# jonaselgammal/GPry

Measured on AMD Instinct MI355X. Metric: gp_refit_plus_nora_acq_cycle_throughput, higher is better.
Workload: dtype f64

## Files before the change

gpry_amd/_lib.py:

```python
import ctypes as C
import ctypes as _ct
import os

import numpy as np

_HERE = os.path.dirname(os.path.abspath(__file__))
LIB_PATH = os.path.join(_HERE, "libgpry_hip.so")

GPRY_MAX_DIM = 32
MASK_CLASSIFIED_INF = 1
MASK_OUTSIDE_TRUST = 2

KERNEL_IDS = {"rbf": 0, "matern12": 1, "matern32": 2, "matern52": 3}
KERNEL_WHITE = 0x10


class GpryAffine(C.Structure):
    _fields_ = [("has_x_affine", C.c_int),
                ("x_lo", C.c_double * GPRY_MAX_DIM),
                ("x_span", C.c_double * GPRY_MAX_DIM),
                ("y_mean", C.c_double), ("y_std", C.c_double),
                ("clip_hi", C.c_double)]


# ... 56 lines not shown
                                + [C.c_int, C.c_int, _vp, _vp]),
    "gpry_maximize_mean": (C.c_int, [_vp, _vp, _vp, _vp, _vp, C.c_int64, _vp, _vp, C.c_int, C.c_int, C.c_double,
                                     C.c_double, C.c_double] + [_vp] * 12 + [_P(C.c_double)]),
    "gpry_maximize_acq": (C.c_int, [_vp, _vp, _vp, _vp, C.c_int64, _vp, _vp, C.c_double, C.c_double, C.c_double, C.c_int,
                                    C.c_int, C.c_double, C.c_double, C.c_double] + [_vp] * 14 + [_P(C.c_double)]),
    "gpry_hessian_mean": (C.c_int, [_vp, _vp, C.c_int64, _vp, _vp, _vp, _P(C.c_double)]),
    "gpry_predict_cov": (C.c_int, [_vp, _vp, C.c_int64, _vp, _vp, _vp, _P(C.c_double)]),
    "gpry_sample_joint": (C.c_int, [_vp, _vp, C.c_int64, _vp, C.c_int64, C.c_uint64, C.c_double, _vp, _vp, _vp, _vp,
                                    _P(C.c_int), _P(C.c_double), _P(C.c_double)]),
    "gpry_loo": (C.c_int, [_vp, _vp, _vp, _vp, _vp, _vp, _P(C.c_double)]),
    "gpry_svm_fit": (C.c_int, [_vp, _vp, _vp, C.c_int64, C.c_int64, C.c_double, C.c_double, C.c_double, C.c_int64, _vp,
                               _P(C.c_double), _P(C.c_double), _P(C.c_double), _P(C.c_int64), _P(C.c_int), _P(C.c_double)]),
    "gpry_leave_out": (C.c_int, [_vp, _vp, _vp, C.c_int64, _vp, _vp, _vp, _vp, _vp, _P(C.c_double)]),
    "gpry_predict_grad": (C.c_int, [_vp, _vp, C.c_int, _vp, _vp, _vp]),
    "gpry_predict_grad_batch": (C.c_int, [_vp, _vp, C.c_int64, C.c_int, _vp, _vp, _vp, _vp]),
    "gpry_predict_point": (C.c_int, [_vp, _vp, C.c_int, C.c_int, _vp, _vp, _vp, _vp, _vp]),
    "gpry_set_gates": (C.c_int, [_vp, _vp, _vp, C.c_int64, C.c_double, C.c_double, C.c_int, _vp]),
    "gpry_sweep_logexp": (C.c_int, [_vp, _vp, C.c_int64, _vp, C.c_double, C.c_double,
                                    C.c_double, _vp, _vp, _vp, _P(C.c_int64)]),
    "gpry_sweep_logexp_given": (C.c_int, [_vp, _vp, C.c_int64, _vp, _vp, _vp, C.c_double, C.c_double,
                                          C.c_double, _vp, _vp, _vp, _P(C.c_int64)]),
    "gpry_sweep_fetch": (C.c_int, [_vp, C.c_int64, _vp, _vp, _vp]),
    "gpry_sweep_prune_info": (C.c_int, [_vp, _vp, _vp]),
    "gpry_sweep_topk": (C.c_int, [_vp, C.c_int64, _vp, C.c_int64, _vp, _P(C.c_int64),
                                  _P(C.c_double)]),
    "gpry_kb_reset": (C.c_int, [_vp]),
    "gpry_kb_register": (C.c_int, [_vp, _vp, C.c_int64, _P(C.c_int64), _vp]),
    "gpry_kb_gram": (C.c_int, [_vp, C.c_int64, _vp, _vp, _P(C.c_int64)]),
    "gpry_kb_gram_rows": (C.c_int, [_vp, _vp, C.c_int64, _vp, _vp, _P(C.c_int64)]),
    "gpry_kb_rank": (C.c_int, [_vp, _vp, C.c_int64, _vp, C.c_int64, _vp, _vp, _vp, _vp, C.c_int64, _vp, C.c_int64, _vp,
                               C.c_int64, _vp, _vp, _vp, _vp, _vp, _P(C.c_int64), _P(C.c_int64), _vp]),
    "gpry_comm_unique_id": (C.c_int, [_vp]),
    "gpry_comm_init": (C.c_int, [_vp, C.c_int, C.c_int, _vp, _P(_vp)]),
    "gpry_comm_destroy": (C.c_int, [_vp]),
    "gpry_comm_info": (C.c_int, [_vp, _P(C.c_int), _P(C.c_int), _P(C.c_int)]),
    "gpry_comm_allgather": (C.c_int, [_vp, _vp, C.c_int64, _vp]),
    "gpry_comm_allreduce_max": (C.c_int, [_vp, _vp, C.c_int64]),
    "gpry_comm_barrier": (C.c_int, [_vp]),
    "gpry_group_create": (C.c_int, [C.c_int, _P(C.c_int), _vp, _P(_vp)]),
    "gpry_group_destroy": (C.c_int, [_vp]),
    "gpry_group_size": (C.c_int, [_vp, _P(C.c_int), _P(C.c_int)]),
    "gpry_group_member": (_vp, [_vp, C.c_int]),
    "gpry_group_last_error": (C.c_char_p, [_vp]),
    "gpry_group_set_model": (C.c_int, [_vp, _vp, _vp, _vp, C.c_int64, C.c_int, C.c_int, _vp,
                                       _P(GpryAffine), _P(C.c_int)]),
    "gpry_group_set_gates": (C.c_int, [_vp, _vp, _vp, C.c_int64, C.c_double, C.c_double, C.c_int, _vp]),
# ... 686 lines not shown
        self._check(self._lib.gpry_sweep_info(self._h, C.byref(form), _ptr(est)), "gpry_sweep_info")
        return {"panel_form": self.PANEL_FORMS.get(form.value, str(form.value)), "panel_error_estimate": float(est[0]),
                "panel_error_mean_worst_case": float(est[1]), "panel_error_variance": float(est[2]), "panel_gate": float(est[3])}

    def sweep_fetch(self, want=("y", "sigma")):
        M = self._sweep_M
        out = {k: (np.empty(M) if k in want else None) for k in ("y", "sigma", "acq")}
        self._check(self._lib.gpry_sweep_fetch(self._h, M, _ptr(out["y"]), _ptr(out["sigma"]),
                                               _ptr(out["acq"])), "gpry_sweep_fetch")
        return out

    PRUNE_INFO = ("pruned", "M", "K_prime", "rounds", "contracted", "completed", "K", "survivors", "y_bound", "live_blocks",
                  "blocks")

    def sweep_prune_info(self):
        info = np.zeros(len(self.PRUNE_INFO), dtype=np.int64)
        dinfo = np.zeros(5)
        self._check(self._lib.gpry_sweep_prune_info(self._h, _ptr(info), _ptr(dinfo)), "gpry_sweep_prune_info")
        out = {k: int(v) for k, v in zip(self.PRUNE_INFO, info)}
        out["tau"] = float(dinfo[0])
        out["stage_ms"] = dict(zip(("sweep_mean", "sweep_prune_select", "sweep_compact", "sweep_prune_gemm"), dinfo[1:].tolist()))
        return out

    def sweep_topk(self, Kp, exclude=None):
        Kp = int(Kp)
        top = np.zeros(max(Kp, 1), dtype=CAND_DTYPE)
        n_out, bound = C.c_int64(0), C.c_double(0.0)
        if exclude is not None and len(exclude):
            exclude = np.ascontiguousarray(np.sort(np.asarray(exclude, dtype=np.int64)))
            nex = len(exclude)
        else:
            exclude, nex = None, 0
        self._check(self._lib.gpry_sweep_topk(self._h, Kp, _ptr(exclude), nex, _ptr(top),
                                              C.byref(n_out), C.byref(bound)), "gpry_sweep_topk")
        return top[:n_out.value], bound.value

    def kb_reset(self):
        self._check(self._lib.gpry_kb_reset(self._h), "gpry_kb_reset")

    def kb_register(self, X, want_var0=True):
        X = _f64(X)
        m = X.shape[0]
        first = C.c_int64(0)
        var0 = np.empty(m) if want_var0 else None
        self._check(self._lib.gpry_kb_register(self._h, _ptr(X), m, C.byref(first), _ptr(var0)),
                    "gpry_kb_register")
# ... 256 lines not shown
```

gpry_amd/csrc/common.h:

```cpp
#pragma once
#include <hip/hip_runtime.h>
#include <stdint.h>
#include <stdio.h>
#include <string.h>
#include <math.h>
#include <string>
#include <vector>
#include <map>

#include "../../include/gpry_hip.h"

#define GPRY_THETA_MAX (2 + GPRY_MAX_DIM)
#define GPRY_BPAR_ROW (2 + GPRY_MAX_DIM)
#define GPRY_BPAR_WHITE (1 + GPRY_MAX_DIM)
#define GPRY_TILE 128
#define GPRY_NB 64

typedef double v4d __attribute__((ext_vector_type(4)));

struct StageTimer {
    double total_ms = 0.0;
    int64_t count = 0;
    std::vector<std::pair<hipEvent_t, hipEvent_t>> pending;
};
// ... 99 lines not shown
    double* dG = nullptr;
    int64_t g_cap = 0;
    double* dsplit = nullptr;
    int64_t split_cap = 0;
    int opt_predict_split = 1;
    int opt_gemm_dma = 1;
    double* dpart = nullptr;
    int64_t part_cap = 0;
    unsigned long long* dkeys = nullptr; int64_t keys_cap = 0;
    unsigned int* dhist = nullptr;
    unsigned int* dselp = nullptr;
    enum { SELP_HIST_WORDS = 12 * 256, SELP_WORDS = 12 * 256 + 12 * 8 };
    int opt_select_fused = 1;
    int opt_prune_one_select = 1;
    int opt_sweep_small_map = 1;
    gpry_cand* dcand = nullptr; int64_t cand_cap = 0;
    unsigned long long* dsel = nullptr;
    enum { DSEL_NAN = 0,
           DSEL_STATE = 0,
           DSEL_EMIT = 4,
           DSEL_SURV = 6,
           DSEL_GIDX = 7,
           DSEL_LIVE = 8,
           DSEL_WORDS = 64 };

    int64_t kb_n = 0, kb_cap = 0;
    int64_t kb_ld = 0;
    double* dU = nullptr;
    double* dXkb = nullptr;
    double* dkbout = nullptr;

    double* dbord = nullptr;
    int64_t bord_cap = 0;
    int64_t n_border = 0;

    void* trtri_plan = nullptr;
    void* trtri_pipe = nullptr;
    int64_t opt_gemm_streamk = 5632;
    int64_t opt_topk_host = 16384;
    int opt_factor_pipeline = 1;
    int opt_factor_pipeline_min = 1280;
    void* chol_plan = nullptr;

    void* srv = nullptr;
    int opt_predict_serve = 1;
    int64_t opt_serve_idle_us = 2000;
    int opt_mcmc_mapped = 0;
    int64_t opt_chol_stacked = 2048;
    int opt_chol_stacked_dense = 0;
    int opt_sweep_overlap = 0;
    int opt_sweep_upload = 1;
    const double* up_X = nullptr;
    const double* up_y = nullptr;
    int up_gates = 0;
    int opt_kb_rank = 1;
    int opt_predict_gates = 0;
    int opt_sweep_prune = 0;
    int opt_sweep_mean_bound = 1;
    int sw_pruned = 0;
    struct PruneState {
        int have_mask = 0;
        int form = 0;
        FinishParams fp = {};
        int64_t n_eval = 0;
        int64_t rounds = 0, evaluated_total = 0, completed = 0, last_K = 0;
        int64_t n_gidx = 0;
        int tau_done = 0;
        double tau = 0.0;
        int64_t survivors = -1;
        int ybound = 0;
        int64_t live_blocks = 0, blocks = 0;
    } prune;
    struct ModelSnap {
        double *dV = nullptr, *dalpha_ = nullptr, *dXs = nullptr, *dX = nullptr;
        int64_t v_cap = 0, a_cap = 0, xs_cap = 0, x_cap = 0;
        int64_t N = 0, Np = 0;
        int d = 0, dpad = 0, kernel_id = 0;
        bool white = false;
        double theta[GPRY_THETA_MAX] = {0};
        gpry_affine tf;
        double xcenter[GPRY_MAX_DIM] = {0};
        bool xs_foreign = false;
    } snap;
    double* dub = nullptr;
    int64_t ub_cap = 0;
    double* dXg = nullptr;
    int64_t xg_cap = 0;
    int64_t* dgidx = nullptr;
    int64_t gidx_cap = 0;
    uint8_t* dmc = nullptr;
    int64_t mc_cap = 0;
    uint8_t* dknn = nullptr;
    int64_t knn_cap = 0;
    uint8_t* dph = nullptr;
// ... 214 lines not shown
```

gpry_amd/csrc/ctx.hip:

```cpp
#include "common.h"
#include <string>
#include <stdarg.h>
#include <dlfcn.h>

thread_local char g_last_error[1024] = {0};
void trtri_plan_free(gpry_ctx* ctx);
void overlap_plan_free(gpry_ctx* ctx);

int gpry_fail(gpry_ctx* ctx, int code, const char* fmt, ...) {
    va_list ap;
    va_start(ap, fmt);
    vsnprintf(g_last_error, sizeof(g_last_error), fmt, ap);
    va_end(ap);
    if (ctx) { strncpy(ctx->err, g_last_error, sizeof(ctx->err) - 1); }
    return code;
}

template <typename T>
int dev_alloc(gpry_ctx* ctx, T** p, int64_t count) {
    *p = nullptr;
    if (count <= 0) count = 1;
    HIP_TRY(ctx, hipMalloc((void**)p, sizeof(T) * (size_t)count));
    return 0;
}
// ... 246 lines not shown
    OPT_INT("gemm_streamk", opt_gemm_streamk, 0, BIG, trtri_plan_free(c)),
    OPT_INT("gemm_small", opt_gemm_small, 0, BIG, c->lml_cache = false),
    OPT_INT("cross_mfma", opt_cross_mfma, 0, 1, (void)0),
    OPT_INT("cross_hybrid", opt_cross_hybrid, 0, 1, (void)0),
    OPT_INT("sweep_chunk", opt_sweep_chunk, 0, BIG, c->opt_sweep_chunk = round_up(c->opt_sweep_chunk, 1024)),
    OPT_INT("topk_host", opt_topk_host, 0, BIG, (void)0),
    OPT_INT("lml_small", opt_lml_small, 0, 1, c->lml_cache = false),
    OPT_INT("lml_cache", opt_lml_cache, 0, 1, c->lml_cache = false),
    OPT_INT("lml_batch", opt_lml_batch, 0, BIG, (void)0),
    OPT_INT("lml_batch_mb", opt_lml_batch_mb, 1, BIG, (void)0),
    OPT_INT("lml_schedule", opt_lml_schedule, 0, 1, (void)0),
    OPT_INT("lml_streams", opt_lml_streams, 1, 8, (void)0),
    OPT_INT("chol_tp_segments", opt_chol_tp_segments, 0, 1, c->lml_cache = false),
    OPT_INT("panel_debug", opt_panel_debug, 0, 511, c->lml_cache = false),
    OPT_INT("tp_left", opt_tp_left, 0, 1, (void)0),
    OPT_INT("tp_block", opt_tp_block, 128, BIG, c->opt_tp_block = round_up(c->opt_tp_block, 128); overlap_plan_free(c)),
    OPT_INT("tp_tail", opt_tp_tail, 128, BIG, c->opt_tp_tail = round_up(c->opt_tp_tail, 128); overlap_plan_free(c)),
    OPT_INT("predict_small", opt_predict_small, 0, BIG, (void)0),
    OPT_INT("predict_split", opt_predict_split, 0, 1, (void)0),
    OPT_INT("sweep_upload", opt_sweep_upload, 0, 1, (void)0),
    OPT_INT("sweep_overlap", opt_sweep_overlap, 0, 1, (void)0),
    OPT_INT("sweep_prune", opt_sweep_prune, 0, 1, (void)0),
    OPT_INT("sweep_mean_bound", opt_sweep_mean_bound, 0, 1, (void)0),
    OPT_INT("sweep_small_map", opt_sweep_small_map, 0, 1, (void)0),
    OPT_INT("select_fused", opt_select_fused, 0, 1, (void)0),
    OPT_INT("prune_one_select", opt_prune_one_select, 0, 1, (void)0),
    OPT_INT("chol_stacked", opt_chol_stacked, 0, BIG, c->lml_cache = false),
    OPT_INT("chol_stacked_dense", opt_chol_stacked_dense, 0, 1, c->lml_cache = false),
    OPT_INT("predict_gates", opt_predict_gates, 0, 1, (void)0),
    OPT_INT("predict_serve", opt_predict_serve, 0, 1, (void)0),
    OPT_INT("serve_idle_us", opt_serve_idle_us, 10, 1000000, (void)0),
    OPT_INT("mcmc_mapped", opt_mcmc_mapped, 0, 1, (void)0),
    OPT_INT("kb_rank", opt_kb_rank, 0, 1, (void)0),
    OPT_INT("svm_iters_per_launch", opt_svm_iters, 1, BIG, (void)0),
};
#undef OPT_INT
const OptionSpec* find_option(const char* key) {
    for (const OptionSpec& o : OPTIONS) if (!strcmp(o.key, key)) return &o;
    return nullptr;
}
}

int gpry_ctx_set_option(gpry_ctx* ctx, const char* key, int64_t value) {
    if (!ctx || !key) return gpry_fail(ctx, -1, "gpry_ctx_set_option: NULL argument");
    GPRY_TRY(serve_stop(ctx));
    const OptionSpec* o = find_option(key);
// ... 374 lines not shown
```

gpry_amd/csrc/kernel_build.hip:

```cpp
#include "common.h"

#include "kern_math.h"

__global__ void scale_train_kernel(const double* __restrict__ X, double* __restrict__ Xs_,
                                   int64_t N, int64_t Np, int d, int dpad, AffParams ap, int* info_,
                                   const double* __restrict__ bpar, int64_t bstride) {
    const int tb = (int)blockIdx.z;
    double* __restrict__ Xs = bset(Xs_, tb, bstride);
    int* info = bset(info_, tb, bstride);
    int64_t idx = (int64_t)blockIdx.x * blockDim.x + threadIdx.x;
    if (idx < 4) info[idx] = 0;
    if (idx >= Np * dpad) return;
    int64_t i = idx / dpad; int k = (int)(idx - i * dpad);
    double v = 0.0;
    if (i < N && k < d) v = X[i * d + k] / (bpar ? bset(bpar, tb, bstride)[1 + k] : ap.ls[k]);
    Xs[idx] = v;
}

int launch_scale_train(gpry_ctx* ctx) {
    AffParams ap = make_ap(ctx, false);
    int64_t n = ctx->Np * ctx->dpad;
    hipLaunchKernelGGL(scale_train_kernel, dim3((unsigned)((n + 255) / 256), 1, (unsigned)ctx->bn), dim3(256), 0,
                       ctx->stream, ctx->dX, ctx->dXs, ctx->N, ctx->Np, ctx->d, ctx->dpad, ap, ctx->dinfo, ctx->bpar, ctx->bstride);
    HIP_TRY(ctx, hipGetLastError());
// ... 223 lines not shown
    for (int jj = nfull; jj < 128; jj++) {
        double v = 0.0;
        if (jj < nvalid) {
            double r2 = 0.0;
#pragma unroll
            for (int k = 0; k < DP; k++) {
                double df = xs[k] - Xl[jj * DP + k];
                r2 = fma(df, df, r2);
            }
            v = kp.C * corr_r2_fast<KID>(r2);
            macc = fma(al[jj], v, macc);
        }
        if (in_chunk && Kst) Kst[((int64_t)jc * 128 + jj) * ldk + ml] = v;
    }
    if (in_chunk && mean_part) mean_part[(int64_t)jc * mc + ml] = macc;
}

template <int DP, int KID, bool HYB, bool BND = false>
__global__ __launch_bounds__(256) void cross_build_mfma_kernel(
    const double* __restrict__ Xcs, int64_t ldm, int64_t mc,
    const double* __restrict__ Ycs, const double* __restrict__ alpha_,
    double* __restrict__ Kst, int64_t ldk, double* __restrict__ mean_part, KernParams kp, double ucut,
    double ubnd = 0.0, double uhi = 0.0, double* __restrict__ sabs_part = nullptr,
    unsigned long long* __restrict__ live_cnt = nullptr) {
    constexpr int S = DP + 2, KS = DP / 4;
    constexpr double SC = corr_scale<KID>();
    __shared__ __attribute__((aligned(16))) double Yl[128 * S];
    __shared__ double yn[128], al[128];
    const int t = threadIdx.x, lane = t & 63, w = t >> 6, r = lane & 15, g = lane >> 4;
    const int jc = blockIdx.y;
    const int64_t mb = (int64_t)blockIdx.x * 256 + 64 * w;
    for (int e = t; e < 128 * (DP / 2); e += 256) {
        const int row = e / (DP / 2), k2 = (e - row * (DP / 2)) * 2;
        *reinterpret_cast<double2*>(Yl + row * S + k2) = *reinterpret_cast<const double2*>(Ycs + ((int64_t)jc * 128 + row) * DP + k2);
    }
    if (t < 128) al[t] = alpha_ ? alpha_[jc * 128 + t] : 0.0;
    double xb[4][KS], xn[4];
#pragma unroll
    for (int tp = 0; tp < 2; tp++) {
        double s0 = 0.0, s1 = 0.0;
#pragma unroll
        for (int kk = 0; kk < KS; kk++) {
            const double2 v = *reinterpret_cast<const double2*>(Xcs + (int64_t)(4 * kk + g) * ldm + mb + 32 * tp + 2 * r);
            xb[2 * tp][kk] = v.x; xb[2 * tp + 1][kk] = v.y;
            s0 = fma(v.x, v.x, s0); s1 = fma(v.y, v.y, s1);
        }
        s0 += __shfl_xor(s0, 16); s0 += __shfl_xor(s0, 32);
        s1 += __shfl_xor(s1, 16); s1 += __shfl_xor(s1, 32);
        xn[2 * tp] = s0 * SC; xn[2 * tp + 1] = s1 * SC;
    }
    __syncthreads();
    if (t < 128) {
        double s = 0.0;
#pragma unroll
        for (int k = 0; k < DP; k++) s = fma(Yl[t * S + k], Yl[t * S + k], s);
        yn[t] = s * SC;
    }
    __syncthreads();
    const int64_t left = kp.N - (int64_t)jc * 128;
    const int nvalid = left >= 128 ? 128 : (left > 0 ? (int)left : 0);
    double macc[4] = {0.0, 0.0, 0.0, 0.0};
    double sacc[4] = {0.0, 0.0, 0.0, 0.0};
    unsigned nlive = 0;
#pragma unroll 1
    for (int j0 = 0; j0 < 128; j0 += 16) {
        double a[KS], ynq[4], alq[4];
#pragma unroll
        for (int kk = 0; kk < KS; kk++) a[kk] = Yl[(j0 + r) * S + 4 * kk + g];
#pragma unroll
        for (int q = 0; q < 4; q++) { ynq[q] = yn[j0 + g + 4 * q]; alq[q] = al[j0 + g + 4 * q]; }
#pragma unroll
        for (int tp = 0; tp < 2; tp++) {
            v4d acc0 = {0.0, 0.0, 0.0, 0.0}, acc1 = {0.0, 0.0, 0.0, 0.0};
#pragma unroll
            for (int kk = 0; kk < KS; kk++) acc0 = __builtin_amdgcn_mfma_f64_16x16x4f64(a[kk], xb[2 * tp][kk], acc0, 0, 0, 0);
#pragma unroll
            for (int kk = 0; kk < KS; kk++) acc1 = __builtin_amdgcn_mfma_f64_16x16x4f64(a[kk], xb[2 * tp + 1][kk], acc1, 0, 0, 0);
            const int64_t mloc = mb + 32 * tp + 2 * r;
            const bool in_chunk = mloc < mc;
            double ue0[4], ue1[4];
            bool live = false;
#pragma unroll
            for (int q = 0; q < 4; q++) {
                ue0[q] = fma(-2.0 * SC, acc0[q], xn[2 * tp] + ynq[q]);
                ue1[q] = fma(-2.0 * SC, acc1[q], xn[2 * tp + 1] + ynq[q]);
                if (BND) live = live || !(ue0[q] >= ubnd && ue0[q] <= uhi) || !(ue1[q] >= ubnd && ue1[q] <= uhi);
            }
            if (BND) {
                if (!__any(live)) continue;
                nlive++;
            }
#pragma unroll
            for (int q = 0; q < 4; q++) {
                const int jj = j0 + g + 4 * q;
                double u0 = ue0[q];
                double u1 = ue1[q];
                if (HYB && (u0 < ucut || u1 < ucut)) {
                    double r0 = 0.0, r1 = 0.0;
#pragma unroll 2
                    for (int k = 0; k < DP; k++) {
                        const double yk = Yl[jj * S + k];
                        const double2 xk = *reinterpret_cast<const double2*>(Xcs + (int64_t)k * ldm + mloc);
                        const double d0 = xk.x - yk, d1 = xk.y - yk;
                        r0 = fma(d0, d0, r0); r1 = fma(d1, d1, r1);
                    }
                    u0 = r0 * SC; u1 = r1 * SC;
                }
                u0 = fmax(u0, 1e-290);
                u1 = fmax(u1, 1e-290);
                double v0 = kp.C * corr_scaled_fast<KID>(u0);
                double v1 = kp.C * corr_scaled_fast<KID>(u1);
                if (jj >= nvalid) { v0 = 0.0; v1 = 0.0; }
// ... 4 lines not shown
                    sacc[2 * tp + 1] = fma(fabs(alq[q]), fabs(v1), sacc[2 * tp + 1]);
                }
                if (in_chunk && Kst) *reinterpret_cast<double2*>(Kst + ((int64_t)jc * 128 + jj) * ldk + mloc) = make_double2(v0, v1);
            }
        }
    }
    if (mean_part) {
#pragma unroll
        for (int tl = 0; tl < 4; tl++) {
            double s = macc[tl];
            s += __shfl_xor(s, 16);
            s += __shfl_xor(s, 32);
            const int64_t ml = mb + 32 * (tl >> 1) + 2 * r + (tl & 1);
            if (g == 0 && ml < mc) mean_part[(int64_t)jc * mc + ml] = s;
            if (BND) {
                double sa = sacc[tl];
                sa += __shfl_xor(sa, 16);
                sa += __shfl_xor(sa, 32);
                if (g == 0 && ml < mc) sabs_part[(int64_t)jc * mc + ml] = sa;
            }
        }
    }
    if (BND && lane == 0 && nlive) atomicAdd(live_cnt, (unsigned long long)nlive);
}
__global__ __launch_bounds__(256) void center_train_kernel(const double* __restrict__ X, double* __restrict__ Ycs, int64_t N, int64_t Np, int d,
                                                           int dsel, AffParams ap, AffParams cen) {
    const int64_t idx = (int64_t)blockIdx.x * blockDim.x + threadIdx.x;
    if (idx >= Np * dsel) return;
    const int64_t i = idx / dsel;
    const int k = (int)(idx - i * dsel);
    Ycs[idx] = (i < N && k < d) ? (X[i * d + k] - cen.lo[k]) / ap.ls[k] : 0.0;
}
__global__ __launch_bounds__(256) void center_cand_kernel(const double* __restrict__ Xc, int64_t M, int64_t m0, int64_t mc, int d, int dsel,
                                                          int has_aff, AffParams ap, AffParams cen, double* __restrict__ Xcs, int64_t ldm) {
    const int64_t idx = (int64_t)blockIdx.x * blockDim.x + threadIdx.x;
    if (idx >= mc * dsel) return;
    const int64_t ml = idx / dsel;
    const int k = (int)(idx - ml * dsel);
    const int64_t m = m0 + ml;
    double v = 0.0;
    if (k < d && m < M) {
        v = Xc[m * d + k];
        if (has_aff) v = (v - ap.lo[k]) / ap.span[k];
        v = (v - cen.lo[k]) / ap.ls[k];
    }
    Xcs[(int64_t)k * ldm + ml] = v;
// ... 40 lines not shown
                            int raw_affine, int hybrid) {
    hipStream_t st = ctx->stream;
    KernParams kp;
    int dsel = 0;
    int64_t ldm = 0;
    GPRY_TRY(center_cands(ctx, Xc, m0, mc, raw_affine, &kp, &dsel, &ldm));
    dim3 grid((unsigned)((mc + 255) / 256), (unsigned)(ctx->Np / 128));
#define CM2(DP, KID) do { const double ucut = 100.0 * corr_scale<KID>();                                                                  \
                       if (hybrid) { hipLaunchKernelGGL((cross_build_mfma_kernel<DP, KID, true>), grid, dim3(256), 0, st, ctx->dXcs, ldm, mc, ctx->dYcs, \
                                                        ctx->dalpha_, Kst, ldk, mean_part, kp, ucut); }                                  \
                       else { hipLaunchKernelGGL((cross_build_mfma_kernel<DP, KID, false>), grid, dim3(256), 0, st, ctx->dXcs, ldm, mc, ctx->dYcs, \
                                                 ctx->dalpha_, Kst, ldk, mean_part, kp, ucut); } } while (0)
#define CM4(KID) { if (dsel == 4) CM2(4, KID); else if (dsel == 8) CM2(8, KID); else if (dsel == 16) CM2(16, KID); \
                   else if (dsel == 24) CM2(24, KID); else CM2(32, KID); }
    DISPATCH_KID(ctx->kernel_id, CM4)
#undef CM4
#undef CM2
    HIP_TRY(ctx, hipGetLastError());
    return 0;
}

int launch_cross_mean_bound(gpry_ctx* ctx, const double* Xc, int64_t m0, int64_t mc, double* mean_part, double* sabs_part,
                            double ubnd, double uhi, unsigned long long* live_cnt) {
    hipStream_t st = ctx->stream;
    KernParams kp;
    int dsel = 0;
    int64_t ldm = 0;
    GPRY_TRY(center_cands(ctx, Xc, m0, mc, 1, &kp, &dsel, &ldm));
    dim3 grid((unsigned)((mc + 255) / 256), (unsigned)(ctx->Np / 128));
#define CB2(DP, KID) hipLaunchKernelGGL((cross_build_mfma_kernel<DP, KID, true, true>), grid, dim3(256), 0, st, ctx->dXcs, ldm, mc, ctx->dYcs, \
                                        ctx->dalpha_, nullptr, mc, mean_part, kp, 100.0 * corr_scale<KID>(), ubnd, uhi, sabs_part, live_cnt)
#define CB4(KID) { if (dsel == 4) CB2(4, KID); else if (dsel == 8) CB2(8, KID); else if (dsel == 16) CB2(16, KID); \
                   else if (dsel == 24) CB2(24, KID); else CB2(32, KID); }
    DISPATCH_KID(ctx->kernel_id, CB4)
#undef CB4
#undef CB2
    HIP_TRY(ctx, hipGetLastError());
    return 0;
}

template <int DP, int KID>
__global__ __launch_bounds__(256) void cross_build_small_kernel(
    const double* __restrict__ Xc, int64_t M, int64_t m0, int64_t mc,
    const double* __restrict__ Xs, const double* __restrict__ alpha_,
    double* __restrict__ Kst, int64_t ldk, double* __restrict__ mean_part,
    KernParams kp, AffParams ap) {
    __shared__ double Xl[128 * DP];
    __shared__ double al[128];
    const int t = threadIdx.x, rg = t >> 6;
    const int64_t ml = (int64_t)blockIdx.x * 64 + (t & 63);
    const int64_t m = m0 + ml;
    const int jc = blockIdx.y;
    for (int e = t; e < 128 * DP; e += 256) {
        int row = e / DP, k = e - row * DP;
// ... 786 lines not shown
```

gpry_amd/csrc/sweep.hip:

```cpp
#include "sweep.h"
#include "acq_math.h"
#include <algorithm>

__global__ void logexp_kernel(const double* __restrict__ mu, const double* __restrict__ sd, int64_t n, double zeta,
                              double baseline, double sigma_n, double* __restrict__ acq) {
    int64_t i = (int64_t)blockIdx.x * blockDim.x + threadIdx.x;
    if (i < n) acq[i] = logexp_value(mu[i], sd[i], zeta, baseline, sigma_n);
}
int launch_logexp(gpry_ctx* ctx, const double* mu, const double* sd, int64_t n, double zeta, double baseline, double sigma_n, double* acq) {
    hipLaunchKernelGGL(logexp_kernel, dim3((unsigned)((n + 255) / 256)), dim3(256), 0, ctx->stream, mu, sd, n, zeta, baseline, sigma_n, acq);
    HIP_TRY(ctx, hipGetLastError());
    return 0;
}

__device__ __forceinline__ double sum_partials(const double* __restrict__ part, int nt, int64_t ldp, int64_t col) {
    double s = 0.0;
#pragma unroll 8
    for (int t = 0; t < nt; t++) s += part[(int64_t)t * ldp + col];
    return s;
}
__device__ __forceinline__ double finish_y(double mu_, unsigned mk, const FinishParams& fp) {
    double y = mu_ * fp.y_std + fp.y_mean;
    y = fmin(y, fp.clip_hi);
    if (mk) y = -INFINITY;
// ... 285 lines not shown

int run_sweep(gpry_ctx* ctx, int64_t M, const SweepRequest& rq) {
    const bool predict = rq.kind == SWEEP_PREDICT, stage_a = rq.kind == SWEEP_STAGE_A, y_given = rq.y_given;
    const int64_t Np = ctx->Np;
    const int nt = (int)(Np / 128);
    const int64_t chunk = sweep_chunk(ctx, M);
    const bool overlap = ctx->opt_sweep_overlap && ctx->stream2 != nullptr && rq.kind == SWEEP_FULL && M > chunk;
    const int nbuf = overlap ? 2 : 1;
    if (stage_a) GPRY_TRY(dev_grow(ctx, &ctx->dub, &ctx->ub_cap, round_up(M, 1024)));
    else GPRY_TRY(dev_grow(ctx, &ctx->dKst, &ctx->kst_cap, nbuf * Np * chunk));
    const bool small_build = predict && M <= 512;
    const int nt_mean = small_build ? 4 * nt : nt;
    const int64_t part_stride = (int64_t)(nt_mean + nt) * chunk;
    GPRY_TRY(ensure_part(ctx, nbuf * part_stride));
    const FinishParams fp = finish_params(ctx, rq);
    ctx->sw_M = M;
    GPRY_TRY(choose_panel_form(ctx, small_build));
    const int form = ctx->panel_form;
    const bool no_panel = stage_a && y_given;
    if (panel_from_matrix_pipe(form) && !no_panel) GPRY_TRY(launch_cross_prepare(ctx));
    if (stage_a) ctx->prune.form = form;
    const MeanBound mb = mean_bound_setup(ctx, rq, fp, nt);
    unsigned long long* live_cnt = nullptr;
    if (stage_a) { ctx->prune.ybound = mb.on ? 1 : 0; ctx->prune.live_blocks = 0; ctx->prune.blocks = 0; }
    if (mb.on) {
        if (!ctx->dsel) GPRY_TRY(dev_alloc(ctx, &ctx->dsel, gpry_ctx::DSEL_WORDS));
        live_cnt = ctx->dsel + gpry_ctx::DSEL_LIVE;
        HIP_TRY(ctx, hipMemsetAsync(live_cnt, 0, 8, ctx->stream));
        if (getenv("GPRY_HIP_DEBUG_PANEL"))
            fprintf(stderr, "gpry: bound pass: u in [%.6g, %.3g] skipped, D %.3g, gamma %.3g\n", mb.ubnd, mb.uhi, mb.D1, mb.g3 / 3.0);
    }
    const double* up_X = ctx->up_X;
    const double* up_y = ctx->up_y;
    const size_t nchunk = (size_t)((M + chunk - 1) / chunk);
    if (up_X || overlap) {
        while (ctx->ev_pool.size() < 3 * nchunk + 1) {
            hipEvent_t ev;
            HIP_TRY(ctx, hipEventCreateWithFlags(&ev, hipEventDisableTiming));
            ctx->ev_pool.push_back(ev);
        }
    }
    const hipStream_t main_stream = ctx->stream, side = ctx->stream2;
    struct StreamSwap {
        gpry_ctx* c; hipStream_t keep;
        StreamSwap(gpry_ctx* ctx, hipStream_t st) : c(ctx), keep(ctx->stream) { c->stream = st; }
        ~StreamSwap() { c->stream = keep; }
    };
    auto upload_chunk = [&](size_t ci, bool gates_on_side) -> int {
        const int64_t m0 = (int64_t)ci * chunk, mc = (M - m0 < chunk) ? M - m0 : chunk;
        HIP_TRY(ctx, hipMemcpyAsync(ctx->dXc + m0 * ctx->d, up_X + m0 * ctx->d, sizeof(double) * mc * ctx->d,
                                    hipMemcpyHostToDevice, side));
// ... 189 lines not shown
    HIP_TRY(ctx, hipMemsetAsync(ctx->dsel + gpry_ctx::DSEL_GIDX, 0, 8, ctx->stream));
    hipLaunchKernelGGL(pruned_idx_kernel, dim3((unsigned)((M + 255) / 256)), dim3(256), 0, ctx->stream, ctx->dsig_all, M, ctx->dgidx, ctx->dsel + gpry_ctx::DSEL_GIDX);
    HIP_TRY(ctx, hipGetLastError());
    unsigned long long n = 0;
    HIP_TRY(ctx, hipMemcpyAsync(&n, ctx->dsel + gpry_ctx::DSEL_GIDX, 8, hipMemcpyDeviceToHost, ctx->stream));
    HIP_TRY(ctx, hipStreamSynchronize(ctx->stream));
    if (n > 0) GPRY_TRY(prune_eval(ctx, (int64_t)n));
    HIP_TRY(ctx, hipStreamSynchronize(ctx->stream));
    ctx->prune.evaluated_total += (int64_t)n;
    ctx->sw_pruned = 0;
    ctx->prune.completed = 1;
    return 0;
}

static int sweep_copy_out(gpry_ctx* ctx, int64_t M, const double* nan_src, unsigned long long* nn, unsigned long long* live,
                          double* y_all, double* sigma_all, double* acq_all) {
    if (nan_src) {
        if (!ctx->dsel) GPRY_TRY(dev_alloc(ctx, &ctx->dsel, gpry_ctx::DSEL_WORDS));
        unsigned long long* dnan = ctx->dsel + gpry_ctx::DSEL_NAN;
        HIP_TRY(ctx, hipMemsetAsync(dnan, 0, 8, ctx->stream));
        hipLaunchKernelGGL(count_nan_kernel, dim3(1024), dim3(256), 0, ctx->stream, nan_src, M, dnan);
        HIP_TRY(ctx, hipMemcpyAsync(nn, dnan, 8, hipMemcpyDeviceToHost, ctx->stream));
    }
    if (live) HIP_TRY(ctx, hipMemcpyAsync(live, ctx->dsel + gpry_ctx::DSEL_LIVE, 8, hipMemcpyDeviceToHost, ctx->stream));
    if (y_all) HIP_TRY(ctx, hipMemcpyAsync(y_all, ctx->dy_all, sizeof(double) * M, hipMemcpyDeviceToHost, ctx->stream));
    if (sigma_all) HIP_TRY(ctx, hipMemcpyAsync(sigma_all, ctx->dsig_all, sizeof(double) * M, hipMemcpyDeviceToHost, ctx->stream));
    if (acq_all) HIP_TRY(ctx, hipMemcpyAsync(acq_all, ctx->dacq_all, sizeof(double) * M, hipMemcpyDeviceToHost, ctx->stream));
    HIP_TRY(ctx, hipStreamSynchronize(ctx->stream));
    return 0;
}

static int sweep_impl(gpry_ctx* ctx, const double* X, int64_t M, const uint8_t* mask, const double* y_given, double zeta,
                      double baseline, double sigma_n, double* y_all, double* sigma_all, double* acq_all, int64_t* n_nan) {
    GPRY_TRY(serve_stop(ctx));
    GPRY_TRY(require_model(ctx, true));
    HIP_TRY(ctx, hipSetDevice(ctx->device));
    if (M <= 0) return gpry_fail(ctx, -1, "sweep: M must be > 0");
    const bool prune = ctx->opt_sweep_prune && !y_all && !sigma_all && !acq_all;
    ctx->sw_pruned = 0;
    const bool piped = X != nullptr && ctx->opt_sweep_upload && ctx->stream2 != nullptr;
    GPRY_TRY(upload_candidates(ctx, piped ? nullptr : X, M, mask, piped));
    SweepRequest rq;
    rq.kind = prune ? SWEEP_STAGE_A : SWEEP_FULL; rq.have_mask = mask != nullptr; rq.y_given = y_given != nullptr;
    rq.zeta = zeta; rq.baseline = baseline; rq.sigma_n = sigma_n;
    if (ctx->gates_on) {
        if (!rq.have_mask) HIP_TRY(ctx, hipMemsetAsync(ctx->dmask, 0, (size_t)M, ctx->stream));
        if (!piped) {
            StageScope s(ctx, "gates");
            GPRY_TRY(launch_gates(ctx, ctx->dXc, M, ctx->dmask));
        }
        rq.have_mask = true;
    }
    struct UploadScope {
        gpry_ctx* c; bool done = false;
        ~UploadScope() {
            c->up_X = nullptr; c->up_y = nullptr; c->up_gates = 0;
            if (!done) { c->sw_M = 0; if (c->stream2) (void)hipStreamSynchronize(c->stream2); (void)hipStreamSynchronize(c->stream); }
        }
    } upload_scope{ctx};
    if (piped) { ctx->up_X = X; ctx->up_gates = ctx->gates_on ? 1 : 0; }
    if (y_given) {
        if (piped) ctx->up_y = y_given;
        else HIP_TRY(ctx, hipMemcpyAsync(ctx->dy_all, y_given, sizeof(double) * M, hipMemcpyHostToDevice, ctx->stream));
    }
    GPRY_TRY(run_sweep(ctx, M, rq));
    unsigned long long nn = 0, live = 0;
    GPRY_TRY(sweep_copy_out(ctx, M, prune ? ctx->dub : ctx->dacq_all, &nn, prune && ctx->prune.ybound ? &live : nullptr,
                            y_all, sigma_all, acq_all));
    upload_scope.done = true;
    if (n_nan) *n_nan = (int64_t)nn;
    if (prune) {
        const int form = ctx->prune.form, ybound = ctx->prune.ybound;
        const int64_t blocks = ctx->prune.blocks;
        ctx->prune = gpry_ctx::PruneState();
        ctx->prune.form = form;
        ctx->prune.ybound = ybound;
        ctx->prune.live_blocks = ybound ? (int64_t)live : 0;
        ctx->prune.blocks = ybound ? blocks : 0;
        ctx->prune.have_mask = rq.have_mask ? 1 : 0;
        ctx->prune.fp = finish_params(ctx, rq);
        GPRY_TRY(prune_snapshot(ctx));
        ctx->sw_pruned = 1;
    }
    return 0;
}

extern "C" {

int gpry_sweep_info(gpry_ctx* ctx, int* panel_form, double* est) {
    if (!ctx) return gpry_fail(nullptr, -1, "gpry_sweep_info: ctx is NULL");
    if (panel_form) *panel_form = ctx->panel_form;
    if (est) for (int k = 0; k < 4; k++) est[k] = ctx->panel_est[k];
    return 0;
}

int gpry_sweep_fetch(gpry_ctx* ctx, int64_t M, double* y_all, double* sigma_all, double* acq_all) {
    if (!ctx) return gpry_fail(nullptr, -1, "gpry_sweep_fetch: ctx is NULL");
    HIP_TRY(ctx, hipSetDevice(ctx->device));
    if (M <= 0 || M != ctx->sw_M) return gpry_fail(ctx, -1, "sweep_fetch: the resident sweep has %lld candidates, not %lld",
                                                  (long long)ctx->sw_M, (long long)M);
// ... 40 lines not shown
```

gpry_amd/csrc/sweep_topk.hip:

```cpp
#include "sweep.h"
#include <algorithm>
#include <functional>

struct SelState { unsigned long long hi; unsigned int lo; unsigned int pad; unsigned long long k_rem; unsigned long long count_ge; };

__device__ __forceinline__ unsigned long long acq_key(double a) {
    unsigned long long b = (unsigned long long)__double_as_longlong(a);
    return (b >> 63) ? ~b : (b | 0x8000000000000000ull);
}

__global__ void make_keys_kernel(const double* __restrict__ acq, int64_t M, unsigned long long* __restrict__ keys) {
    int64_t i = (int64_t)blockIdx.x * blockDim.x + threadIdx.x;
    if (i < M) keys[i] = acq_key(acq[i]);
}
__global__ void exclude_keys_kernel(unsigned long long* keys, const int64_t* excl, int64_t n, int64_t M) {
    int64_t i = (int64_t)blockIdx.x * blockDim.x + threadIdx.x;
    if (i < n && excl[i] >= 0 && excl[i] < M) keys[excl[i]] = 0ull;
}

__device__ __forceinline__ unsigned digit_of(unsigned long long key, unsigned int idx, int pass) {
    return pass < 8 ? (unsigned)((key >> (56 - 8 * pass)) & 0xFF) : (unsigned)((idx >> (24 - 8 * (pass - 8))) & 0xFF);
}
__device__ __forceinline__ bool prefix_match(unsigned long long key, unsigned int idx, const SelState& s, int pass) {
    if (pass == 0) return true;
// ... 460 lines not shown
    if (!info) return gpry_fail(ctx, -1, "sweep_prune_info: info must not be NULL");
    info[0] = ctx->sw_pruned;
    info[1] = ctx->sw_M;
    info[2] = ctx->prune.n_eval;
    info[3] = ctx->prune.rounds;
    info[4] = ctx->prune.evaluated_total;
    info[5] = ctx->prune.completed;
    info[6] = ctx->prune.last_K;
    info[7] = ctx->prune.survivors;
    info[8] = ctx->prune.ybound;
    info[9] = ctx->prune.live_blocks;
    info[10] = ctx->prune.blocks;
    if (dinfo) {
        dinfo[0] = ctx->prune.survivors >= 0 ? ctx->prune.tau : NAN;
        const char* names[] = {"sweep_mean", "sweep_prune_select", "sweep_compact", "sweep_prune_gemm"};
        for (int k = 0; k < 4; k++) {
            double ms = 0.0; int64_t cnt = 0;
            if (gpry_timing_get(ctx, names[k], &ms, &cnt) != 0) ms = 0.0;
            dinfo[1 + k] = ms;
        }
    }
    return 0;
}
```

gpry_amd/gp_acquisition.py:

```python
import os
import inspect
import sys
import warnings
from collections.abc import Mapping
from copy import deepcopy
from functools import partial
from time import time

import numpy as np

import scipy.optimize

import gpry_amd.acquisition_functions as gpryacqfuncs
from gpry_amd.proposal import CentroidsProposer, PartialProposer, Proposer
from gpry_amd.tools import get_Xnumber, get_random_generator, is_in_bounds, remove_0_weight_samples


def builtin_names():
    return [name for name, obj in inspect.getmembers(sys.modules[__name__])
            if inspect.isclass(obj) and issubclass(obj, GenericGPAcquisition)
            and obj is not GenericGPAcquisition]


class NestedSamplerNotInstalledError(Exception):
# ... 687 lines not shown
                 (f"Obtained new MC sample with {self.sampler}" if resample
                  else "Re-evaluated previous MC sample"), level=2)
        t_rank = time()
        self.pool = RankedPool(n_points, gpr=gpr, acq_func=self.acq_func_y_sigma,
                               verbose=self.verbose - 3)
        K = int(self.shortlist_size or max(256, 16 * n_points))
        fed = 0
        with np.errstate(divide="ignore"):
            while True:
                top, bound, exhausted = self._shortlist(gpr, K, exclude)
                new = top[fed:]
                if len(new):
                    self.pool.add(X_dev[new["idx"]], new["y"].copy(), new["sigma"].copy(),
                                  new["acq"].copy(), method="single sort acq")
                fed = len(top)
                if exhausted or self.pool.min_acq >= bound:
                    break
                K *= 4
        self.stats.update(shortlist=fed, cache_models=self.pool.cache_counter,
                          rank_s=time() - t_rank, rank_native=self.pool.rank_native)
        pruned_on = getattr(self, "_pruned_on", [])
        if pruned_on:
            self.stats["prune"] = [t.sweep_prune_info() for t in pruned_on]
        else:
            self.stats.pop("prune", None)
        merged = self.pool.copy(drop_empty=True)
        X_pool, y_pool = merged.X[:n_points], merged.y[:n_points]
        with np.errstate(divide="ignore"):
            acq_pool = self.acq_func_y_sigma(y_pool, merged.sigma[:n_points])
        self._X_already_proposed = np.concatenate([self._X_already_proposed, X_pool])
        self.pool.reset_cache()
        self.log(f"({(time() - t_rank):.2g} sec) Ranked pool of candidates.", level=2)
        return X_pool, y_pool, acq_pool


class _LazyModels(list):

    def __init__(self, session, slot_idx, n_filled):
        super().__init__([None] * len(slot_idx))
        self._session, self._slot_idx, self._n_filled = session, [int(i) for i in slot_idx], n_filled

    def __getitem__(self, i):
        model = super().__getitem__(i)
        if model is None and isinstance(i, (int, np.integer)) and 0 <= i < self._n_filled:
            from gpry_amd.kriging import ConditionedGPR
            model = ConditionedGPR(self._session, self._slot_idx[:i + 1])
# ... 235 lines not shown
```

include/gpry_hip.h:

```cpp
#ifndef GPRY_HIP_H
#define GPRY_HIP_H

#include <stdint.h>

#ifdef __cplusplus
extern "C" {
#endif

typedef struct gpry_ctx gpry_ctx;
typedef struct gpry_comm gpry_comm;
typedef struct gpry_group gpry_group;

enum { GPRY_RBF = 0, GPRY_MATERN12 = 1, GPRY_MATERN32 = 2, GPRY_MATERN52 = 3 };
#define GPRY_KERNEL_WHITE 0x10

#define GPRY_MAX_DIM 32

typedef struct {
    int has_x_affine;
    double x_lo[GPRY_MAX_DIM];
    double x_span[GPRY_MAX_DIM];
    double y_mean, y_std;
    double clip_hi;
} gpry_affine;
// ... 125 lines not shown
                       double* mean_grad, double* kinvk_grad, int* verdict);

int gpry_set_gates(gpry_ctx* ctx, const double* sv, const double* coef, int64_t n_sv, double gamma,
                   double intercept, int positive_is_finite, const double* trust_bounds);

int gpry_svm_fit(gpry_ctx* ctx, const double* X, const uint8_t* finite, int64_t N, int64_t d, double C, double gamma,
                 double eps, int64_t max_iter, double* alpha, double* rho, double* objective, double* violation,
                 int64_t* n_iter, int* status, double* device_ms);

int gpry_sweep_logexp(gpry_ctx* ctx, const double* X, int64_t M, const uint8_t* mask,
                      double zeta, double baseline, double sigma_n,
                      double* y_all, double* sigma_all, double* acq_all,
                      int64_t* n_nan);
int gpry_sweep_logexp_given(gpry_ctx* ctx, const double* X, int64_t M, const uint8_t* mask,
                            const double* y_given, const double* sigma_given,
                            double zeta, double baseline, double sigma_n,
                            double* y_all, double* sigma_all, double* acq_all,
                            int64_t* n_nan);
int gpry_sweep_info(gpry_ctx* ctx, int* panel_form, double* est);
int gpry_sweep_fetch(gpry_ctx* ctx, int64_t M, double* y_all, double* sigma_all, double* acq_all);
int gpry_sweep_topk(gpry_ctx* ctx, int64_t Kp, const int64_t* exclude, int64_t n_exclude,
                    gpry_cand* top, int64_t* n_out, double* bound);
int gpry_sweep_prune_info(gpry_ctx* ctx, int64_t* info, double* dinfo);

int gpry_kb_reset(gpry_ctx* ctx);
int gpry_kb_register(gpry_ctx* ctx, const double* X, int64_t m, int64_t* first,
                     double* var0);
int gpry_kb_gram(gpry_ctx* ctx, int64_t p, double* G, double* kvec, int64_t* n);
int gpry_kb_gram_rows(gpry_ctx* ctx, const int64_t* p, int64_t n_rows, double* G, double* kvec, int64_t* n);
int gpry_kb_rank(gpry_ctx* ctx, const double* X_new, int64_t m_new, double* var0, int64_t n_session,
                 const int64_t* idx, const double* y, const double* sigma, const double* acq, int64_t n_offer,
                 const int64_t* order, int64_t n_order, const double* params, int64_t n_points,
                 int64_t* slot_idx, double* slot_y, double* slot_sigma, double* slot_acq, double* slot_acq_cond,
                 int64_t* cache_counter, int64_t* info, int64_t* stats);

int gpry_comm_unique_id(uint8_t id[128]);
int gpry_comm_init(gpry_ctx* ctx, int world, int rank, const uint8_t id[128],
                   gpry_comm** out);
int gpry_comm_destroy(gpry_comm* comm);
int gpry_comm_info(gpry_comm* comm, int* world, int* rank, int* device);
int gpry_comm_allgather(gpry_comm* comm, const void* send, int64_t bytes, void* recv);
int gpry_comm_allreduce_max(gpry_comm* comm, double* inout, int64_t n);
int gpry_comm_barrier(gpry_comm* comm);

int gpry_group_create(int n, const int* devices, gpry_ctx* adopt0, gpry_group** out);
int gpry_group_destroy(gpry_group* group);
// ... 39 lines not shown
```

Measured before the change: 62.98 million.

## Screen cross-mean bound tiles with fp32 MFMA before exact fp64 pass

Adds a screening step to the bound-pruning cross-build kernel. It computes the squared distances in fp32 MFMA using rigorous error margins, and skips the fp64 MFMA and the exp work for 16x32 tiles whose distances all fall certifiably inside the skip interval. The saving targets the fp64 matrix cost on tiles that would be discarded anyway. In exchange it uses extra LDS and registers for fp32 copies and adds a second counter and an info API. Occupancy may drop, and the screen is wasted work whenever it fails to certify a tile.

Result: faster. 65.49 million, median of 6 (+4.0%).

```diff
diff --git a/gpry_amd/_lib.py b/gpry_amd/_lib.py
--- a/gpry_amd/_lib.py
+++ b/gpry_amd/_lib.py
@@ -102,6 +102,7 @@
                                           C.c_double, _vp, _vp, _vp, _P(C.c_int64)]),
     "gpry_sweep_fetch": (C.c_int, [_vp, C.c_int64, _vp, _vp, _vp]),
     "gpry_sweep_prune_info": (C.c_int, [_vp, _vp, _vp]),
+    "gpry_sweep_screen_info": (C.c_int, [_vp, _vp]),
     "gpry_sweep_topk": (C.c_int, [_vp, C.c_int64, _vp, C.c_int64, _vp, _P(C.c_int64),
                                   _P(C.c_double)]),
     "gpry_kb_reset": (C.c_int, [_vp]),
@@ -834,6 +835,11 @@
         out["stage_ms"] = dict(zip(("sweep_mean", "sweep_prune_select", "sweep_compact", "sweep_prune_gemm"), dinfo[1:].tolist()))
         return out
 
+    def sweep_screen_info(self):
+        out = np.zeros(2, dtype=np.int64)
+        self._check(self._lib.gpry_sweep_screen_info(self._h, _ptr(out)), "gpry_sweep_screen_info")
+        return {"certified": int(out[0]), "blocks": int(out[1])}
+
     def sweep_topk(self, Kp, exclude=None):
         Kp = int(Kp)
         top = np.zeros(max(Kp, 1), dtype=CAND_DTYPE)
diff --git a/gpry_amd/csrc/common.h b/gpry_amd/csrc/common.h
--- a/gpry_amd/csrc/common.h
+++ b/gpry_amd/csrc/common.h
@@ -145,6 +145,7 @@
            DSEL_SURV = 6,
            DSEL_GIDX = 7,
            DSEL_LIVE = 8,
+           DSEL_FALL = 9,
            DSEL_WORDS = 64 };
 
     int64_t kb_n = 0, kb_cap = 0;
@@ -180,6 +181,7 @@
     int opt_predict_gates = 0;
     int opt_sweep_prune = 0;
     int opt_sweep_mean_bound = 1;
+    int opt_sweep_screen = 1;
     int sw_pruned = 0;
     struct PruneState {
         int have_mask = 0;
@@ -193,6 +195,7 @@
         int64_t survivors = -1;
         int ybound = 0;
         int64_t live_blocks = 0, blocks = 0;
+        int64_t cert_blocks = 0;
     } prune;
     struct ModelSnap {
         double *dV = nullptr, *dalpha_ = nullptr, *dXs = nullptr, *dX = nullptr;
diff --git a/gpry_amd/csrc/ctx.hip b/gpry_amd/csrc/ctx.hip
--- a/gpry_amd/csrc/ctx.hip
+++ b/gpry_amd/csrc/ctx.hip
@@ -292,6 +292,7 @@
     OPT_INT("sweep_overlap", opt_sweep_overlap, 0, 1, (void)0),
     OPT_INT("sweep_prune", opt_sweep_prune, 0, 1, (void)0),
     OPT_INT("sweep_mean_bound", opt_sweep_mean_bound, 0, 1, (void)0),
+    OPT_INT("sweep_screen", opt_sweep_screen, 0, 1, (void)0),
     OPT_INT("sweep_small_map", opt_sweep_small_map, 0, 1, (void)0),
     OPT_INT("select_fused", opt_select_fused, 0, 1, (void)0),
     OPT_INT("prune_one_select", opt_prune_one_select, 0, 1, (void)0),
diff --git a/gpry_amd/csrc/kernel_build.hip b/gpry_amd/csrc/kernel_build.hip
--- a/gpry_amd/csrc/kernel_build.hip
+++ b/gpry_amd/csrc/kernel_build.hip
@@ -269,20 +269,26 @@
     const double* __restrict__ Ycs, const double* __restrict__ alpha_,
     double* __restrict__ Kst, int64_t ldk, double* __restrict__ mean_part, KernParams kp, double ucut,
     double ubnd = 0.0, double uhi = 0.0, double* __restrict__ sabs_part = nullptr,
-    unsigned long long* __restrict__ live_cnt = nullptr) {
+    unsigned long long* __restrict__ live_cnt = nullptr, int screen = 0) {
+    typedef float v4f __attribute__((ext_vector_type(4)));
     constexpr int S = DP + 2, KS = DP / 4;
     constexpr double SC = corr_scale<KID>();
     __shared__ __attribute__((aligned(16))) double Yl[128 * S];
     __shared__ double yn[128], al[128];
+    constexpr int SF = DP + 1;
+    __shared__ float Yf[BND ? 128 * SF : 1];
     const int t = threadIdx.x, lane = t & 63, w = t >> 6, r = lane & 15, g = lane >> 4;
     const int jc = blockIdx.y;
     const int64_t mb = (int64_t)blockIdx.x * 256 + 64 * w;
     for (int e = t; e < 128 * (DP / 2); e += 256) {
         const int row = e / (DP / 2), k2 = (e - row * (DP / 2)) * 2;
-        *reinterpret_cast<double2*>(Yl + row * S + k2) = *reinterpret_cast<const double2*>(Ycs + ((int64_t)jc * 128 + row) * DP + k2);
+        const double2 v = *reinterpret_cast<const double2*>(Ycs + ((int64_t)jc * 128 + row) * DP + k2);
+        *reinterpret_cast<double2*>(Yl + row * S + k2) = v;
+        if (BND) { Yf[row * SF + k2] = (float)v.x; Yf[row * SF + k2 + 1] = (float)v.y; }
     }
     if (t < 128) al[t] = alpha_ ? alpha_[jc * 128 + t] : 0.0;
     double xb[4][KS], xn[4];
+    float xbf[4][KS];
 #pragma unroll
     for (int tp = 0; tp < 2; tp++) {
         double s0 = 0.0, s1 = 0.0;
@@ -290,6 +296,7 @@
         for (int kk = 0; kk < KS; kk++) {
             const double2 v = *reinterpret_cast<const double2*>(Xcs + (int64_t)(4 * kk + g) * ldm + mb + 32 * tp + 2 * r);
             xb[2 * tp][kk] = v.x; xb[2 * tp + 1][kk] = v.y;
+            if (BND) { xbf[2 * tp][kk] = (float)v.x; xbf[2 * tp + 1][kk] = (float)v.y; }
             s0 = fma(v.x, v.x, s0); s1 = fma(v.y, v.y, s1);
         }
         s0 += __shfl_xor(s0, 16); s0 += __shfl_xor(s0, 32);
@@ -308,16 +315,67 @@
     const int nvalid = left >= 128 ? 128 : (left > 0 ? (int)left : 0);
     double macc[4] = {0.0, 0.0, 0.0, 0.0};
     double sacc[4] = {0.0, 0.0, 0.0, 0.0};
-    unsigned nlive = 0;
+    unsigned nlive = 0, nfall = 0;
+    bool scr = false;
+    float lo32 = 0.0f, hi32 = 0.0f;
+    if (BND && screen) {
+        const double y0 = yn[lane], y1 = yn[lane + 64];
+        bool bad = !(y0 <= 1e36) || !(y1 <= 1e36);
+        double ym = fmax(y0, y1), xm = fmax(fmax(xn[0], xn[1]), fmax(xn[2], xn[3]));
+#pragma unroll
+        for (int tl = 0; tl < 4; tl++) bad = bad || !(xn[tl] <= 1e36);
+#pragma unroll
+        for (int o = 1; o < 64; o <<= 1) { ym = fmax(ym, __shfl_xor(ym, o)); xm = fmax(xm, __shfl_xor(xm, o)); }
+        const double rs = sqrt(ym) + sqrt(xm);
+        const double delta = 5.9604644775390625e-08 * (double)(kp.d + 8) * rs * rs;
+        const double lo = ubnd + delta, hi = uhi - delta;
+        lo32 = (float)lo;
+        if ((double)lo32 < lo) lo32 = __uint_as_float(__float_as_uint(lo32) + 1u);
+        hi32 = (float)hi;
+        if ((double)hi32 > hi) hi32 = __uint_as_float(__float_as_uint(hi32) - 1u);
+        scr = !__any(bad || !(hi > 0.0) || !(lo32 <= hi32));
+        lo32 = __uint_as_float(__builtin_amdgcn_readfirstlane(__float_as_uint(lo32)));
+        hi32 = __uint_as_float(__builtin_amdgcn_readfirstlane(__float_as_uint(hi32)));
+    }
 #pragma unroll 1
     for (int j0 = 0; j0 < 128; j0 += 16) {
         double a[KS], ynq[4], alq[4];
-#pragma unroll
-        for (int kk = 0; kk < KS; kk++) a[kk] = Yl[(j0 + r) * S + 4 * kk + g];
-#pragma unroll
-        for (int q = 0; q < 4; q++) { ynq[q] = yn[j0 + g + 4 * q]; alq[q] = al[j0 + g + 4 * q]; }
+        if (!BND) {
+#pragma unroll
+            for (int kk = 0; kk < KS; kk++) a[kk] = Yl[(j0 + r) * S + 4 * kk + g];
+#pragma unroll
+            for (int q = 0; q < 4; q++) { ynq[q] = yn[j0 + g + 4 * q]; alq[q] = al[j0 + g + 4 * q]; }
+        }
 #pragma unroll
         for (int tp = 0; tp < 2; tp++) {
+            if (BND && scr) {
+                float af[KS];
+                double yns[4];
+#pragma unroll
+                for (int kk = 0; kk < KS; kk++) af[kk] = Yf[(j0 + r) * SF + 4 * kk + g];
+#pragma unroll
+                for (int i = 0; i < 4; i++) yns[i] = yn[j0 + 4 * g + i];
+                v4f c0 = {0.0f, 0.0f, 0.0f, 0.0f}, c1 = {0.0f, 0.0f, 0.0f, 0.0f};
+#pragma unroll
+                for (int kk = 0; kk < KS; kk++) {
+                    c0 = __builtin_amdgcn_mfma_f32_16x16x4f32(af[kk], xbf[2 * tp][kk], c0, 0, 0, 0);
+                    c1 = __builtin_amdgcn_mfma_f32_16x16x4f32(af[kk], xbf[2 * tp + 1][kk], c1, 0, 0, 0);
+                }
+                float mn = __builtin_inff(), mx = -__builtin_inff();
+#pragma unroll
+                for (int i = 0; i < 4; i++) {
+                    const float w0 = fmaf(-2.0f * (float)SC, c0[i], (float)(xn[2 * tp] + yns[i]));
+                    const float w1 = fmaf(-2.0f * (float)SC, c1[i], (float)(xn[2 * tp + 1] + yns[i]));
+                    mn = fminf(mn, fminf(w0, w1)); mx = fmaxf(mx, fmaxf(w0, w1));
+                }
+                if (!__any(!(mn >= lo32 && mx <= hi32))) continue;
+            }
+            if (BND) {
+#pragma unroll
+                for (int kk = 0; kk < KS; kk++) a[kk] = Yl[(j0 + r) * S + 4 * kk + g];
+#pragma unroll
+                for (int q = 0; q < 4; q++) { ynq[q] = yn[j0 + g + 4 * q]; alq[q] = al[j0 + g + 4 * q]; }
+            }
             v4d acc0 = {0.0, 0.0, 0.0, 0.0}, acc1 = {0.0, 0.0, 0.0, 0.0};
 #pragma unroll
             for (int kk = 0; kk < KS; kk++) acc0 = __builtin_amdgcn_mfma_f64_16x16x4f64(a[kk], xb[2 * tp][kk], acc0, 0, 0, 0);
@@ -334,7 +392,7 @@
                 if (BND) live = live || !(ue0[q] >= ubnd && ue0[q] <= uhi) || !(ue1[q] >= ubnd && ue1[q] <= uhi);
             }
             if (BND) {
-                if (!__any(live)) continue;
+                if (!__any(live)) { if (screen) nfall++; continue; }
                 nlive++;
             }
 #pragma unroll
@@ -385,6 +443,7 @@
         }
     }
     if (BND && lane == 0 && nlive) atomicAdd(live_cnt, (unsigned long long)nlive);
+    if (BND && lane == 0 && nfall) atomicAdd(live_cnt + 1, (unsigned long long)nfall);
 }
 __global__ __launch_bounds__(256) void center_train_kernel(const double* __restrict__ X, double* __restrict__ Ycs, int64_t N, int64_t Np, int d,
                                                            int dsel, AffParams ap, AffParams cen) {
@@ -471,6 +530,7 @@
 
 int launch_cross_mean_bound(gpry_ctx* ctx, const double* Xc, int64_t m0, int64_t mc, double* mean_part, double* sabs_part,
                             double ubnd, double uhi, unsigned long long* live_cnt) {
+    const int screen = ctx->opt_sweep_screen;
     hipStream_t st = ctx->stream;
     KernParams kp;
     int dsel = 0;
@@ -478,7 +538,7 @@
     GPRY_TRY(center_cands(ctx, Xc, m0, mc, 1, &kp, &dsel, &ldm));
     dim3 grid((unsigned)((mc + 255) / 256), (unsigned)(ctx->Np / 128));
 #define CB2(DP, KID) hipLaunchKernelGGL((cross_build_mfma_kernel<DP, KID, true, true>), grid, dim3(256), 0, st, ctx->dXcs, ldm, mc, ctx->dYcs, \
-                                        ctx->dalpha_, nullptr, mc, mean_part, kp, 100.0 * corr_scale<KID>(), ubnd, uhi, sabs_part, live_cnt)
+                                        ctx->dalpha_, nullptr, mc, mean_part, kp, 100.0 * corr_scale<KID>(), ubnd, uhi, sabs_part, live_cnt, screen)
 #define CB4(KID) { if (dsel == 4) CB2(4, KID); else if (dsel == 8) CB2(8, KID); else if (dsel == 16) CB2(16, KID); \
                    else if (dsel == 24) CB2(24, KID); else CB2(32, KID); }
     DISPATCH_KID(ctx->kernel_id, CB4)
diff --git a/gpry_amd/csrc/sweep.hip b/gpry_amd/csrc/sweep.hip
--- a/gpry_amd/csrc/sweep.hip
+++ b/gpry_amd/csrc/sweep.hip
@@ -331,11 +331,11 @@
     if (stage_a) ctx->prune.form = form;
     const MeanBound mb = mean_bound_setup(ctx, rq, fp, nt);
     unsigned long long* live_cnt = nullptr;
-    if (stage_a) { ctx->prune.ybound = mb.on ? 1 : 0; ctx->prune.live_blocks = 0; ctx->prune.blocks = 0; }
+    if (stage_a) { ctx->prune.ybound = mb.on ? 1 : 0; ctx->prune.live_blocks = 0; ctx->prune.blocks = 0; ctx->prune.cert_blocks = 0; }
     if (mb.on) {
         if (!ctx->dsel) GPRY_TRY(dev_alloc(ctx, &ctx->dsel, gpry_ctx::DSEL_WORDS));
         live_cnt = ctx->dsel + gpry_ctx::DSEL_LIVE;
-        HIP_TRY(ctx, hipMemsetAsync(live_cnt, 0, 8, ctx->stream));
+        HIP_TRY(ctx, hipMemsetAsync(live_cnt, 0, 16, ctx->stream));
         if (getenv("GPRY_HIP_DEBUG_PANEL"))
             fprintf(stderr, "gpry: bound pass: u in [%.6g, %.3g] skipped, D %.3g, gamma %.3g\n", mb.ubnd, mb.uhi, mb.D1, mb.g3 / 3.0);
     }
@@ -571,7 +571,7 @@
         hipLaunchKernelGGL(count_nan_kernel, dim3(1024), dim3(256), 0, ctx->stream, nan_src, M, dnan);
         HIP_TRY(ctx, hipMemcpyAsync(nn, dnan, 8, hipMemcpyDeviceToHost, ctx->stream));
     }
-    if (live) HIP_TRY(ctx, hipMemcpyAsync(live, ctx->dsel + gpry_ctx::DSEL_LIVE, 8, hipMemcpyDeviceToHost, ctx->stream));
+    if (live) HIP_TRY(ctx, hipMemcpyAsync(live, ctx->dsel + gpry_ctx::DSEL_LIVE, 16, hipMemcpyDeviceToHost, ctx->stream));
     if (y_all) HIP_TRY(ctx, hipMemcpyAsync(y_all, ctx->dy_all, sizeof(double) * M, hipMemcpyDeviceToHost, ctx->stream));
     if (sigma_all) HIP_TRY(ctx, hipMemcpyAsync(sigma_all, ctx->dsig_all, sizeof(double) * M, hipMemcpyDeviceToHost, ctx->stream));
     if (acq_all) HIP_TRY(ctx, hipMemcpyAsync(acq_all, ctx->dacq_all, sizeof(double) * M, hipMemcpyDeviceToHost, ctx->stream));
@@ -613,8 +613,8 @@
         else HIP_TRY(ctx, hipMemcpyAsync(ctx->dy_all, y_given, sizeof(double) * M, hipMemcpyHostToDevice, ctx->stream));
     }
     GPRY_TRY(run_sweep(ctx, M, rq));
-    unsigned long long nn = 0, live = 0;
-    GPRY_TRY(sweep_copy_out(ctx, M, prune ? ctx->dub : ctx->dacq_all, &nn, prune && ctx->prune.ybound ? &live : nullptr,
+    unsigned long long nn = 0, live[2] = {0, 0};
+    GPRY_TRY(sweep_copy_out(ctx, M, prune ? ctx->dub : ctx->dacq_all, &nn, prune && ctx->prune.ybound ? live : nullptr,
                             y_all, sigma_all, acq_all));
     upload_scope.done = true;
     if (n_nan) *n_nan = (int64_t)nn;
@@ -624,7 +624,8 @@
         ctx->prune = gpry_ctx::PruneState();
         ctx->prune.form = form;
         ctx->prune.ybound = ybound;
-        ctx->prune.live_blocks = ybound ? (int64_t)live : 0;
+        ctx->prune.live_blocks = ybound ? (int64_t)live[0] : 0;
+        ctx->prune.cert_blocks = ybound && ctx->opt_sweep_screen ? blocks - (int64_t)live[0] - (int64_t)live[1] : 0;
         ctx->prune.blocks = ybound ? blocks : 0;
         ctx->prune.have_mask = rq.have_mask ? 1 : 0;
         ctx->prune.fp = finish_params(ctx, rq);
diff --git a/gpry_amd/csrc/sweep_topk.hip b/gpry_amd/csrc/sweep_topk.hip
--- a/gpry_amd/csrc/sweep_topk.hip
+++ b/gpry_amd/csrc/sweep_topk.hip
@@ -506,3 +506,11 @@
     }
     return 0;
 }
+
+extern "C" int gpry_sweep_screen_info(gpry_ctx* ctx, int64_t out[2]) {
+    if (!ctx) return gpry_fail(nullptr, -1, "gpry_sweep_screen_info: ctx is NULL");
+    if (!out) return gpry_fail(ctx, -1, "sweep_screen_info: out must not be NULL");
+    out[0] = ctx->prune.cert_blocks;
+    out[1] = ctx->prune.blocks;
+    return 0;
+}
diff --git a/gpry_amd/gp_acquisition.py b/gpry_amd/gp_acquisition.py
--- a/gpry_amd/gp_acquisition.py
+++ b/gpry_amd/gp_acquisition.py
@@ -733,6 +733,9 @@
         pruned_on = getattr(self, "_pruned_on", [])
         if pruned_on:
             self.stats["prune"] = [t.sweep_prune_info() for t in pruned_on]
+            for t, st in zip(pruned_on, self.stats["prune"]):
+                if hasattr(t, "sweep_screen_info"):
+                    st["certified"] = t.sweep_screen_info()["certified"]
         else:
             self.stats.pop("prune", None)
         merged = self.pool.copy(drop_empty=True)
diff --git a/include/gpry_hip.h b/include/gpry_hip.h
--- a/include/gpry_hip.h
+++ b/include/gpry_hip.h
@@ -171,6 +171,7 @@
 int gpry_sweep_topk(gpry_ctx* ctx, int64_t Kp, const int64_t* exclude, int64_t n_exclude,
                     gpry_cand* top, int64_t* n_out, double* bound);
 int gpry_sweep_prune_info(gpry_ctx* ctx, int64_t* info, double* dinfo);
+int gpry_sweep_screen_info(gpry_ctx* ctx, int64_t out[2]);
 
 int gpry_kb_reset(gpry_ctx* ctx);
 int gpry_kb_register(gpry_ctx* ctx, const double* X, int64_t m, int64_t* first,
```
